# wearable-motion-capture/arm-pose-estimation

Measured on AMD Instinct MI355X. Metric: IMU windows/sec, higher is better.
Workload: dtype f32; 1 GPU; BASELINE configs[2]: watch_phone_pocket_lstm path, 1024 windows/GPU x 64 frames x 22 features (I=22,H=256,L=2,O=14), z-score+LSTM+head+denorm+FK, inputs resident in HBM; windows_per_gpu=1024, frames=64, features=22

## Files before the change

arm-pose-estimation_amd/csrc/lstm_cluster32.hip:

```cpp
#include <type_traits>

#include "ape_internal.h"
#include "async_look.h"
#include "../../include/ape_hip.h"

namespace {

typedef float f32x16 __attribute__((ext_vector_type(16)));
typedef unsigned u32x4 __attribute__((__vector_size__(4 * sizeof(unsigned))));
constexpr unsigned SPIN_LIMIT = 1u << 22;

#ifdef APE_CLUSTER_STAMPS
#define C32_TL(i) do { if (p.dbg_wg != nullptr && tid == 0 && cluster == 0 && member == 0 && (i) < 200) p.dbg_wg[256 + (i)] = __builtin_readcyclecounter(); } while (0)
#else
#define C32_TL(i) do {} while (0)
#endif

__device__ __forceinline__ float sigm(float v) { return __builtin_amdgcn_rcpf(1.0f + __builtin_amdgcn_exp2f(-1.4426950408889634f * v)); }
__device__ __forceinline__ float tanh_(float v) { return 2.0f * __builtin_amdgcn_rcpf(1.0f + __builtin_amdgcn_exp2f(-2.885390081777927f * v)) - 1.0f; }

template <bool AG>
__device__ __forceinline__ void mfma32(f32x16& acc, float w, float a) {
    if constexpr (AG) asm volatile("v_mfma_f32_32x32x2_f32 %0, %1, %2, %0" : "+v"(acc) : "a"(w), "v"(a));
    else asm volatile("v_mfma_f32_32x32x2_f32 %0, %1, %2, %0" : "+v"(acc) : "v"(w), "v"(a));
}
__device__ __forceinline__ void mfma_drain(f32x16& acc) { asm volatile("s_nop 15\n\ts_nop 7" : "+v"(acc)); }
template <bool AG>
__device__ __forceinline__ void mfma16(f32x16& acc, const u32x4& w, const u32x4& b) {
    if constexpr (AG) asm volatile("v_mfma_f32_32x32x16_f16 %0, %1, %2, %0" : "+v"(acc) : "a"(w), "v"(b));
    else asm volatile("v_mfma_f32_32x32x16_f16 %0, %1, %2, %0" : "+v"(acc) : "v"(w), "v"(b));
}

template <int NB, bool AG, int NW, typename Mid>
__device__ __forceinline__ void span32(f32x16& acc, const float* __restrict__ src, int stride, const float (&w)[NW], int w0, Mid&& mid) {
    f32x4 a0 = *reinterpret_cast<const f32x4*>(src);
    f32x4 a1 = (NB > 1) ? *reinterpret_cast<const f32x4*>(src + stride) : a0;
    f32x4 a2 = a1;
#pragma unroll
    for (int kb = 0; kb < NB; ++kb) {
        if (kb + 2 < NB) a2 = *reinterpret_cast<const f32x4*>(src + stride * (kb + 2));
#pragma unroll
        for (int j = 0; j < 4; ++j) mfma32<AG>(acc, w[w0 + 4 * kb + j], a0[j]);
        mid(kb);
        a0 = a1;
        a1 = a2;
    }
}

template <int NS, bool AG, int NG, typename Mid>
__device__ __forceinline__ void span16(f32x16& acc, const float* __restrict__ src, const u32x4 (&w)[NG], int g0, Mid&& mid) {
    constexpr int SL = 2 * 2 * 32 * 4;
    u32x4 h0 = *reinterpret_cast<const u32x4*>(src), l0 = *reinterpret_cast<const u32x4*>(src + 128);
    u32x4 h1 = (NS > 1) ? *reinterpret_cast<const u32x4*>(src + SL) : h0, l1 = (NS > 1) ? *reinterpret_cast<const u32x4*>(src + SL + 128) : l0;
    u32x4 h2 = h1, l2 = l1;
#pragma unroll
    for (int s = 0; s < NS; ++s) {
        if (s + 2 < NS) {
            h2 = *reinterpret_cast<const u32x4*>(src + SL * (s + 2));
            l2 = *reinterpret_cast<const u32x4*>(src + SL * (s + 2) + 128);
        }
        mfma16<AG>(acc, w[g0 + 2 * s], h0);
        mfma16<AG>(acc, w[g0 + 2 * s], l0);
        mid(2 * s);
        mfma16<AG>(acc, w[g0 + 2 * s + 1], h0);
        mid(2 * s + 1);
        h0 = h1; l0 = l1;
        h1 = h2; l1 = l2;
    }
}

template <bool HOT>
__device__ __forceinline__ void dma_1k(unsigned lds_addr, unsigned voff, u32x4 rsrc, unsigned soff, int piece_bytes) {
    if constexpr (HOT) {
        unsigned tmp;
        asm volatile("s_add_i32 m0, %1, %5\n\ts_add_i32 %0, %4, %5\n\tbuffer_load_dwordx4 %2, %3, %0 offen sc1 lds"
                     : "=&s"(tmp) : "s"(lds_addr), "v"(voff), "s"(rsrc), "s"(soff), "i"(piece_bytes) : "memory");
    } else {
        asm volatile("s_mov_b32 m0, %0\n\ts_nop 3\n\tbuffer_load_dwordx4 %1, %2, %3 offen sc1 lds"
                     :: "s"(lds_addr + (unsigned)piece_bytes), "v"(voff), "s"(rsrc), "s"(soff + (unsigned)piece_bytes) : "memory");
    }
}


#ifndef C32_QF
#define C32_QF 3
#endif
#ifndef C32_QPD
#define C32_QPD 0
#endif
#ifndef C32_XS
#define C32_XS 1
#endif
#ifndef C32_QFP
#define C32_QFP 12
#endif
#ifndef C32_QPX
#define C32_QPX 33
#endif
#ifndef C32_QJX
#define C32_QJX 54
#endif
#if defined(APE_C32_COUNTS) && defined(APE_C32_WAITS)
#error "APE_C32_COUNTS and APE_C32_WAITS write the same words of dbg_wg: one build, one of them"
#endif
template <int H, int L, int KX, bool ENDS, int BXU>
__global__ __launch_bounds__(256, 1) void ape_lstm_cluster32(const ClusterParams p) {
    constexpr int UPW = 8;
    constexpr int GH = H / (4 * UPW);
    constexpr int MR = 32;
    constexpr int SX = KX + 4;
    constexpr int BX = KX / 8, BH = H / 8;
    constexpr int NW0 = 4 * (BX + BH);
    constexpr int NW1 = 4 * (2 * BH);
    constexpr int NFL = 4 * GH;
    constexpr int HL = GH * 4 * MR * 8;
    constexpr int NDMA = HL * 4 / 1024 / 4;
    static_assert(H == 256 && L == 2 && KX == 32 && GH == 8 && NDMA == 8, "built for the 2 x 256 models");
    static_assert(BXU == BX || (BXU == BX - 1 && !ENDS), "the short-window instantiation keeps the four-block input span");

    const int tid = threadIdx.x;
    const int lane = tid & 63;
    const int wave = __builtin_amdgcn_readfirstlane(tid >> 6);
    const int n = lane & 31, hh = lane >> 5;
    const int T = p.T, I = p.I, O = p.O;
    const bool normalize = (p.flags & APE_FLAG_NORMALIZE_INPUT) != 0;
    const bool bcast_x = (p.flags & APE_FLAG_BROADCAST_X) != 0;

    extern __shared__ __attribute__((aligned(16))) float smem[];
    float* hb0 = smem;
    float* hb1 = hb0 + 2 * HL;
    float* xin = hb1 + HL;
    f32x4* bias_s = reinterpret_cast<f32x4*>(xin + 2 * MR * SX);
    f32x4* park_s = bias_s + 4 * L * 4 * 64;
    unsigned* look_s = reinterpret_cast<unsigned*>(park_s + 4 * 4 * 64);
    int* ctl = reinterpret_cast<int*>(look_s + 4 * 64);

    unsigned* const class_ticket = p.xcc_slots + 64;
    unsigned* const xcc_words = p.xcc_slots + 64 + 8 * 16;
    const int cls = blockIdx.x & 7;
    unsigned my_xcc;
    asm volatile("s_getreg_b32 %0, hwreg(HW_REG_XCC_ID)" : "=s"(my_xcc));
    my_xcc &= 0xFu;
    if (tid == 0) {
        ctl[0] = 0;
        ctl[1] = -1;
        if (__hip_atomic_load(p.status, __ATOMIC_RELAXED, __HIP_MEMORY_SCOPE_AGENT) == 0u) {
            const unsigned tk = __hip_atomic_fetch_add(class_ticket + cls * 16, 1u, __ATOMIC_RELAXED, __HIP_MEMORY_SCOPE_AGENT);
            if (tk < gridDim.x / 8) ctl[1] = (int)tk;
            else __hip_atomic_store(p.status, 2u, __ATOMIC_RELAXED, __HIP_MEMORY_SCOPE_AGENT);
        }
    }
    __syncthreads();
    if (ctl[1] < 0) return;
    const int ticket = __builtin_amdgcn_readfirstlane(ctl[1]);
    const int cluster = (ticket / GH) * 8 + cls, member = ticket % GH;
    const int row0 = cluster * MR;
    C32_TL(0);
    if (tid == 0)
        __hip_atomic_store(xcc_words + cluster * GH + member, 0x10u | my_xcc, __ATOMIC_RELAXED, __HIP_MEMORY_SCOPE_AGENT);

    constexpr int NE = (MR * KX) / 256;
    const int xk = tid % KX, xrow = tid / KX;
    const int rows_here = bcast_x ? MR : max(0, min(MR, p.B - row0));
    const unsigned long long x_addr = reinterpret_cast<unsigned long long>(p.x + (bcast_x ? (size_t)0 : (size_t)row0 * T * I));
    const unsigned x_lo = __builtin_amdgcn_readfirstlane((unsigned)x_addr), x_hi = __builtin_amdgcn_readfirstlane((unsigned)(x_addr >> 32));
    const int x_bytes = __builtin_amdgcn_readfirstlane((int)((size_t)(bcast_x ? 1 : rows_here) * T * I * sizeof(float)));
    const __amdgpu_buffer_rsrc_t x_rsrc = __builtin_amdgcn_make_buffer_rsrc(
        reinterpret_cast<float*>(((unsigned long long)x_hi << 32) | x_lo), 0, x_bytes, 0x00020000);
    const unsigned x_rowbytes = bcast_x ? 0u : (unsigned)(T * I * sizeof(float));
    const unsigned x_off0 = (xk < I) ? (unsigned)xrow * x_rowbytes + (unsigned)(xk * sizeof(float)) : 0x80000000u;
    const unsigned x_estride = (unsigned)(256 / KX) * x_rowbytes;
    float xr[NE];
    auto fetch_x = [&](int t) {
        const int slot = (t + p.x_ring >= T) ? t + p.x_ring - T : t + p.x_ring;
#pragma unroll
        for (int e = 0; e < NE; ++e) {
            const unsigned off = (xrow + e * (256 / KX) < rows_here) ? x_off0 + (unsigned)e * x_estride : 0x80000000u;
            xr[e] = __builtin_bit_cast(float, __builtin_amdgcn_raw_buffer_load_b32(x_rsrc, off, (unsigned)(slot * I * sizeof(float)), 0));
        }
    };
    double x_mean = (normalize && xk < I) ? p.xx_m[xk] : 0.0;
    double x_std = (normalize && xk < I) ? p.xx_s[xk] : 1.0;
    double x_rstd = (normalize && xk < I) ? p.xx_r[xk] : 1.0;
    asm volatile("" : "+v"(x_mean), "+v"(x_std), "+v"(x_rstd));
    auto stage_x = [&](int t) {
        float* const dst = xin + (ENDS ? 0 : (t & 1) * (MR * SX));
#pragma unroll
        for (int e = 0; e < NE; ++e) {
            const double d = (double)xr[e] - x_mean;
            const double q0 = d * x_rstd;
            const double rr = fma(-q0, x_std, d);
            const double q1 = fma(rr, x_rstd, q0);
            dst[(xrow + e * (256 / KX)) * SX + xk] = (float)((rr == rr) ? q1 : q0);
        }
    };
    constexpr int XA = ENDS ? 0 : 1;
    fetch_x(0);

    float w0[4 * BXU];
    u32x4 w0h[NW0 / 4 - BX];
    u32x4 w1[NW1 / 4];
    const f32x4* const s0 = reinterpret_cast<const f32x4*>(p.wcl[0]) + ((size_t)(member * 4 + wave) * (NW0 / 4)) * 64 + lane;
    const u32x4* const s1 = reinterpret_cast<const u32x4*>(p.wcl[1]) + ((size_t)(member * 4 + wave) * (NW1 / 4)) * 64 + lane;
#pragma unroll
    for (int i = 0; i < BXU; ++i) {
        const f32x4 v = s0[i * 64];
        w0[4 * i] = v[0]; w0[4 * i + 1] = v[1]; w0[4 * i + 2] = v[2]; w0[4 * i + 3] = v[3];
    }
    auto load_weights = [&]() {
#pragma unroll
        for (int i = BX; i < NW0 / 4; ++i) w0h[i - BX] = reinterpret_cast<const u32x4*>(s0)[i * 64];
#pragma unroll
        for (int i = 0; i < NW1 / 4; ++i) w1[i] = s1[i * 64];
    };
#pragma unroll
    for (int l = 0; l < L; ++l)
#pragma unroll
        for (int gate = 0; gate < 4; ++gate) {
            f32x4 bv;
#pragma unroll
            for (int j = 0; j < 4; ++j) bv[j] = p.bias[l][gate * H + member * 32 + wave * 8 + 4 * hh + j] * p.gate_scale[l];
            bias_s[((wave * L + l) * 4 + gate) * 64 + lane] = bv;
        }
    float cst[L][4];
#pragma unroll
    for (int l = 0; l < L; ++l)
#pragma unroll
        for (int j = 0; j < 4; ++j) cst[l][j] = 0.0f;

    const __amdgpu_buffer_rsrc_t hx_rsrc = __builtin_amdgcn_make_buffer_rsrc(p.hx, 0, (int)p.hx_bytes, 0x00020000);
    const unsigned long long hx_addr = reinterpret_cast<unsigned long long>(p.hx);
    u32x4 hx_desc;
    hx_desc[0] = __builtin_amdgcn_readfirstlane((unsigned)hx_addr);
    hx_desc[1] = __builtin_amdgcn_readfirstlane((unsigned)(hx_addr >> 32) & 0xFFFFu);
    hx_desc[2] = __builtin_amdgcn_readfirstlane((unsigned)p.hx_bytes);
    hx_desc[3] = 0x00020000u;
    unsigned* const flags_of = p.xflags + (size_t)cluster * L * NFL;
    const ape_desc_t fl_desc = ape_make_desc(p.xflags, (unsigned)((gridDim.x / GH) * L * NFL * sizeof(unsigned)));
    const unsigned fl_off = (unsigned)(cluster * L * NFL * sizeof(unsigned));
    const unsigned look_voff = (unsigned)((lane & (NFL - 1)) * sizeof(unsigned));
    const unsigned look_lds = (unsigned)reinterpret_cast<unsigned long long>(look_s) + (unsigned)(wave * 256);
    const unsigned* const look_mine = look_s + wave * 64 + lane;
    constexpr unsigned SET_BYTES = HL * sizeof(float);
    auto hx_base = [&](int l, int par) -> unsigned { return (unsigned)((((size_t)cluster * L + l) * 2 + par) * SET_BYTES); };
    const unsigned hb0_lds = (unsigned)reinterpret_cast<unsigned long long>(hb0);
    const unsigned hb1_lds = (unsigned)reinterpret_cast<unsigned long long>(hb1);

    stage_x(0);
    if (T > 1) fetch_x(1);

    if (wave == 0) {
        unsigned spins = 0, v = 0u;
        while (true) {
            v = 0x10u | my_xcc;
            if (lane < GH) v = __hip_atomic_load(xcc_words + cluster * GH + lane, __ATOMIC_RELAXED, __HIP_MEMORY_SCOPE_AGENT);
            if (__all((int)(v != 0u))) break;
            if (++spins > SPIN_LIMIT || __hip_atomic_load(p.status, __ATOMIC_RELAXED, __HIP_MEMORY_SCOPE_AGENT) != 0u) {
                if (lane == 0) {
                    ctl[0] = 1;
                    __hip_atomic_store(p.status, 1u, __ATOMIC_RELAXED, __HIP_MEMORY_SCOPE_AGENT);
                }
                break;
            }
            __builtin_amdgcn_s_sleep(2);
        }
        const int same = __all((int)((v & 0xFu) == my_xcc));
        if (lane == 0) ctl[3] = same;
    }
    __syncthreads();
    if (ctl[0] != 0) return;
    C32_TL(1);
    const bool in_l2 = APE_HANDOVER_IN_L2(p.flags, ctl[3] != 0);

    auto wait_flags = [&](int l, unsigned want) {
        unsigned spins = 0;
        while (true) {
            unsigned v = want;
            if (lane < NFL) v = __hip_atomic_load(flags_of + l * NFL + lane, __ATOMIC_RELAXED, __HIP_MEMORY_SCOPE_AGENT);
            if (__all((int)(v >= want))) return;
            if (++spins > SPIN_LIMIT || __hip_atomic_load(p.status, __ATOMIC_RELAXED, __HIP_MEMORY_SCOPE_AGENT) != 0u) {
                if (lane == 0) {
                    ctl[0] = 1;
                    __hip_atomic_store(p.status, 1u, __ATOMIC_RELAXED, __HIP_MEMORY_SCOPE_AGENT);
                }
                return;
            }
            __builtin_amdgcn_s_sleep(1);
        }
    };
    const unsigned dma_voff = (unsigned)(lane * 16);
    auto opaque = [](unsigned v) -> unsigned { asm volatile("" : "+s"(v)); return v; };
    const unsigned wave_kib = (unsigned)(wave * 1024);
    auto issue_piece = [&](auto hot_tag, int l, int step, int k) {
        constexpr bool HOT = decltype(hot_tag)::value;
        const unsigned wk = HOT ? wave_kib : opaque(wave_kib);
        const unsigned src = hx_base(l, step & 1) + wk;
        const unsigned dst = (l == 0 ? hb0_lds + (unsigned)((step & 1) * SET_BYTES) : hb1_lds) + wk;
        dma_1k<HOT>(dst, dma_voff, hx_desc, src, k * 4096);
    };
    constexpr std::true_type HOT{};
    constexpr std::false_type COLD{};
    int pend_idx = -1;
    unsigned pend_epoch = 0u;
    auto raise_pending = [&]() {
        if (pend_idx < 0) return;
        if (lane == 0) __hip_atomic_store(flags_of + pend_idx, pend_epoch, __ATOMIC_RELAXED, __HIP_MEMORY_SCOPE_AGENT);
        pend_idx = -1;
    };
    auto bar = [&]() { asm volatile("s_waitcnt lgkmcnt(0)\n\ts_barrier" ::: "memory"); };

    auto cell_update = [&](const f32x16& acc, int l, float (&c_)[4], float (&hn)[4]) {
        const float ks = -1.4426950408889634f * p.gate_descale[l], kt = -2.885390081777927f * p.gate_descale[l];
#pragma unroll
        for (int j = 0; j < 4; j += 2) {
            typedef float f32x2 __attribute__((ext_vector_type(2)));
            auto exp2_2 = [](f32x2 v) { return f32x2{__builtin_amdgcn_exp2f(v[0]), __builtin_amdgcn_exp2f(v[1])}; };
            auto rcp_2 = [](f32x2 v) { return f32x2{__builtin_amdgcn_rcpf(v[0]), __builtin_amdgcn_rcpf(v[1])}; };
            const f32x2 ai = {acc[j], acc[j + 1]}, af = {acc[4 + j], acc[5 + j]}, ag = {acc[8 + j], acc[9 + j]}, ao = {acc[12 + j], acc[13 + j]};
            const f32x2 iv = rcp_2(1.0f + exp2_2(ks * ai));
            const f32x2 fv = rcp_2(1.0f + exp2_2(ks * af));
            const f32x2 gv = 2.0f * rcp_2(1.0f + exp2_2(kt * ag)) - 1.0f;
            const f32x2 ov = rcp_2(1.0f + exp2_2(ks * ao));
            const f32x2 c = fv * f32x2{c_[j], c_[j + 1]} + iv * gv;
            c_[j] = c[0]; c_[j + 1] = c[1];
            const f32x2 h = ov * (2.0f * rcp_2(1.0f + exp2_2(-2.885390081777927f * c)) - 1.0f);
            hn[j] = h[0]; hn[j + 1] = h[1];
        }
    };
    const unsigned pub_off = (unsigned)((((member * 4 + wave) * MR + n) * 8 + 4 * hh) * sizeof(float));
    const unsigned pub_off_split = (unsigned)(((member * 4 + wave) * 2 * MR + hh * MR + n) * 16);
    auto split_h = [&](const float (&h)[4]) -> u32x4 {
        unsigned hw[2], lw[2];
#pragma unroll
        for (int d = 0; d < 2; ++d) {
            const float a = h[2 * d] * (float)(1 << APE_C32_HSHIFT), b = h[2 * d + 1] * (float)(1 << APE_C32_HSHIFT);
            const _Float16 ah = (_Float16)a, bh = (_Float16)b;
            const _Float16 al = (_Float16)(a - (float)ah), bl = (_Float16)(b - (float)bh);
            hw[d] = (unsigned)__builtin_bit_cast(unsigned short, ah) | ((unsigned)__builtin_bit_cast(unsigned short, bh) << 16);
            lw[d] = (unsigned)__builtin_bit_cast(unsigned short, al) | ((unsigned)__builtin_bit_cast(unsigned short, bl) << 16);
        }
        u32x4 r;
#pragma unroll
        for (int d = 0; d < 2; ++d) {
            const auto sw = __builtin_amdgcn_permlane32_swap(hw[d], lw[d], false, false);
            r[d] = sw[0];
            r[2 + d] = sw[1];
        }
        return r;
    };

    if constexpr (!ENDS) {
        if (1 < T) {
            stage_x(1);
            if (2 < T) fetch_x(2);
        }
        load_weights();
    } else {
        f32x16 acc;
#pragma unroll
        for (int gate = 0; gate < 4; ++gate) {
            const f32x4 bv = bias_s[((wave * L + 0) * 4 + gate) * 64 + lane];
            acc[4 * gate] = bv[0]; acc[4 * gate + 1] = bv[1]; acc[4 * gate + 2] = bv[2]; acc[4 * gate + 3] = bv[3];
        }
        span32<BXU, false, 4 * BXU>(acc, xin + n * SX + hh * 4, 8, w0, 0, [&](int) {});
        mfma_drain(acc);
        float h0[4];
        cell_update(acc, 0, cst[0], h0);
        const u32x4 hv = split_h(h0);
        if (in_l2) __builtin_amdgcn_raw_buffer_store_b128(hv, hx_rsrc, hx_base(0, 0) + pub_off_split, 0, 0);
        else __builtin_amdgcn_raw_buffer_store_b128(hv, hx_rsrc, hx_base(0, 0) + pub_off_split, 0, 16 );
        asm volatile("s_waitcnt vmcnt(0)" ::: "memory");
        if (lane == 0) __hip_atomic_store(flags_of + member * 4 + wave, 1u, __ATOMIC_RELAXED, __HIP_MEMORY_SCOPE_AGENT);
        asm volatile("" ::: "memory");
        load_weights();
        bar();
        if (1 < T) {
            stage_x(1);
            if (2 < T) fetch_x(2);
        }
    }
    C32_TL(2);

    const int P = T + L - 1;
    bool prefetched = false;
    bool parked = false;
#ifdef APE_C32_COUNTS
    unsigned lc_block[2] = {0u, 0u}, lc_go[2] = {0u, 0u}, lc_n[2] = {0u, 0u};
    unsigned long long lc_top[2] = {0ull, 0ull}, lc_t0 = 0ull;
    const unsigned long long lc_start = __builtin_amdgcn_s_memtime();
#endif
#ifdef APE_C32_WAITS
    unsigned long long lw[4] = {0ull, 0ull, 0ull, 0ull}, lw_t0 = 0ull;
    unsigned lw_n[3] = {0u, 0u, 0u};
    const unsigned long long lw_start = __builtin_amdgcn_s_memtime();
#define C32_WAIT_T0() do { if (ST) lw_t0 = __builtin_amdgcn_s_memtime(); } while (0)
#define C32_WAIT_T1(k) do { if (ST) lw[k] += __builtin_amdgcn_s_memtime() - lw_t0; } while (0)
#else
#define C32_WAIT_T0() do {} while (0)
#define C32_WAIT_T1(k) do {} while (0)
#endif
#ifdef APE_CLUSTER_STAMPS
    unsigned long long dg_block[2] = {0, 0}, dg_go[2] = {0, 0};
    unsigned long long dgh[2][6] = {};
    unsigned long long dgc[2][5] = {};
    auto now = [&]() -> unsigned long long {
        const unsigned long long c = __builtin_readcyclecounter();
        asm volatile("s_waitcnt lgkmcnt(0)" ::: "memory");
        return c;
    };
#endif
    auto section = [&](auto steady_tag, auto layer_tag, auto mode_tag, const int ph) -> bool {
        constexpr bool ST = decltype(steady_tag)::value;
        constexpr int l = decltype(layer_tag)::value;
        constexpr int MODE = decltype(mode_tag)::value;
        static_assert(MODE == 0 || (l == L - 1 && (MODE == 3 || !ST)), "the special forms are layer 1's");
        const int t = ph - l;
        const bool active = ST || (t >= 0 && t < T);
        const bool need = ST || (t >= 1 && t <= T);
#ifdef APE_CLUSTER_STAMPS
        const unsigned long long c0 = ST ? now() : 0ull;
#endif
#ifdef APE_C32_COUNTS
        lc_t0 = __builtin_amdgcn_s_memtime();
#endif
        if constexpr (MODE != 3) C32_WAIT_T0();
        if (MODE == 3) {
        } else if (need) {
            if (!prefetched) {
#ifdef APE_CLUSTER_STAMPS
                dg_block[l] += 1;
#endif
#ifdef APE_C32_COUNTS
                lc_block[l] += 1u;
#endif
                asm volatile("s_waitcnt vmcnt(0)" ::: "memory");
                raise_pending();
                wait_flags(l, (unsigned)t);
#pragma unroll
                for (int k = 0; k < NDMA; ++k) issue_piece(COLD, l, t - 1, k);
                asm volatile("s_waitcnt vmcnt(0)" ::: "memory");
            } else {
                asm volatile("s_waitcnt vmcnt(1)" ::: "memory");
            }
        }
        prefetched = false;
#ifdef APE_CLUSTER_STAMPS
        const unsigned long long c1 = ST ? now() : 0ull;
#endif
        if constexpr (MODE != 3) bar();
#ifdef APE_CLUSTER_STAMPS
        const unsigned long long c2 = ST ? now() : 0ull;
#endif
#ifdef APE_C32_COUNTS
        if (ST && MODE != 3) { lc_top[l] += __builtin_amdgcn_s_memtime() - lc_t0; lc_n[l] += 1u; }
#endif
#ifdef APE_C32_WAITS
        if constexpr (MODE != 3) { C32_WAIT_T1(3); if (ST) lw_n[1] += 1u; }
#endif
        const int abort_word = (MODE == 3) ? 0 : ctl[0];
        C32_TL(8 + 2 * (2 * ph + l));
        constexpr int ln = (l + 1 < L) ? l + 1 : 0;
        const int tn = (l + 1 < L) ? t - 1 : t + L;
        const bool pre = (l == L - 1) && (ST || (tn >= 1 && tn <= T));
        unsigned peek = (unsigned)tn;
        bool go = false;
        constexpr int NBL = (l == 0) ? BXU + BH : 2 * BH;
        constexpr bool LW = ST && !ENDS && MODE == 3;
        constexpr bool XS = LW && C32_XS != 0;
        constexpr int QF = (!ENDS && l == 0 && C32_XS != 0) ? (ST ? BXU + C32_QFP : (C32_QF > BXU ? C32_QF : BXU)) : C32_QF;
        constexpr int QP = (MODE == 1) ? 16 : LW ? C32_QPX : NBL / 2 - 2 + C32_QPD, QJ = (MODE == 1) ? 20 : LW ? C32_QJX : NBL / 2 + 2 + C32_QPD;
        static_assert(!LW || (QP >= 0 && QP < QJ - 1 && QJ + NDMA <= 2 * BH), "the look, its judge and the eight pieces fit the section");
        bool staged = false;
#ifdef APE_CLUSTER_STAMPS
        unsigned long long hk0 = 0, hk_free = 0;
#define HK_BEGIN() do { if (ST) hk0 = now(); } while (0)
#define HK_END(k) do { if (ST) dgh[l][k] += now() - hk0; } while (0)
#else
#define HK_BEGIN() do {} while (0)
#define HK_END(k) do {} while (0)
#endif
        auto mid = [&](int q) {
#ifdef APE_CLUSTER_STAMPS
            if (ST && q == QF + 2) hk_free = now();
            if (ST && q == QF + 10) dgh[l][5] += now() - hk_free;
#endif
            if (!XS && q == QF) {
                HK_BEGIN();
                asm volatile("s_waitcnt vmcnt(0)" ::: "memory");
                raise_pending();
                HK_END(0);
            }
            if (l == L - 1 && q == ((MODE == 3) ? BH + 1 : QF + 1) && (ST || ph + 1 + XA < T)) {
                HK_BEGIN();
                stage_x(ph + 1 + XA);
                if (ST || ph + 2 + XA < T) fetch_x(ph + 2 + XA);
                staged = true;
                HK_END(1);
            }
            if constexpr (l == L - 1) {
                if (q == QP) look_issue(look_lds, look_voff, fl_desc, fl_off + (unsigned)(ln * NFL * sizeof(unsigned)));
                if (q == QJ - 1) {
                    C32_WAIT_T0();
                    look_landed();
                    C32_WAIT_T1(1);
                    peek = *look_mine;
                }
                if (q == QJ) {
                    HK_BEGIN();
                    go = pre && __all((int)(peek >= (unsigned)tn)) != 0;
                    HK_END(2);
                }
                if (q >= QJ && q < QJ + NDMA && go) {
                    HK_BEGIN();
                    issue_piece(HOT, ln, tn - 1, q - QJ);
                    HK_END(3);
                }
            }
        };
        float hnew[4] = {0.0f, 0.0f, 0.0f, 0.0f};
        if (active) {
            if constexpr (XS) {
                look_issue(look_lds, look_voff, fl_desc, fl_off + (unsigned)(l * NFL * sizeof(unsigned)));
                f32x16 ax;
#pragma unroll
                for (int gate = 0; gate < 4; ++gate) {
                    const f32x4 bv = bias_s[((wave * L + 0) * 4 + gate) * 64 + lane];
                    ax[4 * gate] = bv[0]; ax[4 * gate + 1] = bv[1]; ax[4 * gate + 2] = bv[2]; ax[4 * gate + 3] = bv[3];
                }
                span32<BXU, false, 4 * BXU>(ax, xin + ((ph + 1) & 1) * (MR * SX) + n * SX + hh * 4, 8, w0, 0, [&](int) {});
                mfma_drain(ax);
#pragma unroll
                for (int gate = 0; gate < 4; ++gate)
                    park_s[(wave * 4 + gate) * 64 + lane] = f32x4{ax[4 * gate], ax[4 * gate + 1], ax[4 * gate + 2], ax[4 * gate + 3]};
                parked = true;
            }
            bool from_park = false;
            if constexpr (l == 0 && !ENDS) {
                from_park = parked;
                parked = false;
            }
            const f32x4* const start_s = from_park ? park_s + wave * 4 * 64 + lane : bias_s + (wave * L + l) * 4 * 64 + lane;
            f32x16 acc;
#pragma unroll
            for (int gate = 0; gate < 4; ++gate) {
                const f32x4 bv = start_s[gate * 64];
                acc[4 * gate] = bv[0]; acc[4 * gate + 1] = bv[1]; acc[4 * gate + 2] = bv[2]; acc[4 * gate + 3] = bv[3];
            }
            const int frag = hh * 2 * MR * 4 + n * 4;
            if constexpr (l == 0) {
                if (!from_park) span32<BXU, false, 4 * BXU>(acc, xin + (ENDS ? 0 : (t & 1) * (MR * SX)) + n * SX + hh * 4, 8, w0, 0, [&](int q) { mid(q); });
                if (ST || t > 0) span16<BH / 2, false, NW0 / 4 - BX>(acc, hb0 + ((t - 1) & 1) * HL + frag, w0h, 0, [&](int q) { mid(BXU + q); });
            } else if constexpr (MODE == 3) {
                constexpr int QO = QF + 1, QO2 = QO + 12;
                static_assert(XS || (QO2 + 4 + NDMA <= QP && (LW || QP < BH)), "the own gather's hooks sit in front of the look for the next section");
                unsigned pk = (unsigned)t;
                bool got1 = false, got2 = false;
                if constexpr (XS) {
                    C32_WAIT_T0();
                    look_landed();
                    C32_WAIT_T1(0);
                    raise_pending();
                    pk = *look_mine;
                    got1 = __all((int)(pk >= (unsigned)t)) != 0;
                    span16<BH / 2, true, NW1 / 4>(acc, hb0 + (t & 1) * HL + frag, w1, 0, [&](int q) {
                        mid(q);
                        if (q < NDMA && got1) issue_piece(HOT, l, t - 1, q);
                    });
                } else
                span16<BH / 2, true, NW1 / 4>(acc, hb0 + (t & 1) * HL + frag, w1, 0, [&](int q) {
                    mid(q);
                    if (q == QO) look_issue(look_lds, look_voff, fl_desc, fl_off + (unsigned)(l * NFL * sizeof(unsigned)));
                    if (q == QO + 3) {
                        C32_WAIT_T0();
                        look_landed();
                        C32_WAIT_T1(0);
                        pk = *look_mine;
                    }
                    if (q == QO + 4) got1 = __all((int)(pk >= (unsigned)t)) != 0;
                    if (q >= QO + 4 && q < QO + 4 + NDMA && got1) issue_piece(HOT, l, t - 1, q - (QO + 4));
                    if constexpr (!ST) {
                        if (q == QO2 && !got1) look_issue(look_lds, look_voff, fl_desc, fl_off + (unsigned)(l * NFL * sizeof(unsigned)));
                        if (q == QO2 + 3 && !got1) {
                            look_landed();
                            pk = *look_mine;
                        }
                        if (q == QO2 + 4 && !got1) got2 = __all((int)(pk >= (unsigned)t)) != 0;
                        if (q >= QO2 + 4 && q < QO2 + 4 + NDMA && got2) issue_piece(HOT, l, t - 1, q - (QO2 + 4));
                    }
                });
#ifdef APE_C32_COUNTS
                lc_t0 = __builtin_amdgcn_s_memtime();
#endif
                C32_WAIT_T0();
                if (!got1 && !got2) {
#ifdef APE_C32_WAITS
                    if (ST) lw_n[2] += 1u;
#endif
#ifdef APE_CLUSTER_STAMPS
                    dg_block[l] += 1;
#endif
#ifdef APE_C32_COUNTS
                    lc_block[l] += 1u;
#endif
                    asm volatile("s_waitcnt vmcnt(0)" ::: "memory");
                    raise_pending();
                    wait_flags(l, (unsigned)t);
#pragma unroll
                    for (int k = 0; k < NDMA; ++k) issue_piece(COLD, l, t - 1, k);
                }
                asm volatile("s_waitcnt vmcnt(0)" ::: "memory");
                bar();
#ifdef APE_C32_COUNTS
                if (ST) { lc_top[l] += __builtin_amdgcn_s_memtime() - lc_t0; lc_n[l] += 1u; }
#endif
#ifdef APE_C32_WAITS
                C32_WAIT_T1(2);
                if (ST) lw_n[0] += 1u;
#endif
                if (ctl[0] != 0) return false;
                span16<BH / 2, true, NW1 / 4>(acc, hb1 + frag, w1, BH, [&](int q) { mid(BH + q); });
            } else {
                span16<BH / 2, true, NW1 / 4>(acc, hb0 + (t & 1) * HL + frag, w1, 0, [&](int q) { mid(q); });
                if (ST || t > 0) span16<BH / 2, true, NW1 / 4>(acc, hb1 + frag, w1, BH, [&](int q) { mid(BH + q); });
            }
#ifdef APE_CLUSTER_STAMPS
            const unsigned long long c3 = ST ? now() : 0ull;
            if (ST) { dgc[l][0] += c1 - c0; dgc[l][1] += c2 - c1; dgc[l][2] += c3 - c2; }
#endif
            mfma_drain(acc);
            cell_update(acc, l, cst[l], hnew);
        }
        if (abort_word != 0) return false;
        if (!ST && pend_idx >= 0) {
            asm volatile("s_waitcnt vmcnt(0)" ::: "memory");
            raise_pending();
        }
        if (go) prefetched = true;
#ifdef APE_CLUSTER_STAMPS
        if (go) dg_go[ln] += 1;
#endif
#ifdef APE_C32_COUNTS
        if (go) lc_go[ln] += 1u;
#endif
        if constexpr (l == L - 1) {
            if (!ST && !staged && ph + 1 + XA < T) {
                stage_x(ph + 1 + XA);
                if (ph + 2 + XA < T) fetch_x(ph + 2 + XA);
            }
        }
        {
            const bool head_only = (l == L - 1) && !ST && t == T - 1;
            const u32x4 hs = split_h(hnew);
            const u32x4 hv = head_only ? u32x4{__builtin_bit_cast(unsigned, hnew[0]), __builtin_bit_cast(unsigned, hnew[1]),
                                               __builtin_bit_cast(unsigned, hnew[2]), __builtin_bit_cast(unsigned, hnew[3])} : hs;
            const unsigned off = active ? hx_base(l, t & 1) + (head_only ? pub_off : pub_off_split) : 0x80000000u;
            if (in_l2) __builtin_amdgcn_raw_buffer_store_b128(hv, hx_rsrc, off, 0, 0);
            else __builtin_amdgcn_raw_buffer_store_b128(hv, hx_rsrc, off, 0, 16 );
            if (active) {
                pend_idx = l * NFL + member * 4 + wave;
                pend_epoch = (unsigned)(t + 1);
            }
        }
#ifdef APE_CLUSTER_STAMPS
        if (ST) { dgc[l][3] += now() - c2; dgc[l][4] += 1; }
#endif
        C32_TL(9 + 2 * (2 * ph + l));
        return true;
    };
    bool ok = true;
#pragma unroll 1
    for (int ph = ENDS ? 1 : 0; ph < P && ok; ++ph) {
        const bool st0 = ph >= 2 && ph <= T - 3, st1 = st0;
        using M0 = std::integral_constant<int, 0>;
        using L0 = std::integral_constant<int, 0>;
        using L1 = std::integral_constant<int, 1>;
        ok = st0 ? section(std::true_type{}, L0{}, M0{}, ph) : section(std::false_type{}, L0{}, M0{}, ph);
        if (!ok) break;
        const int t1 = ph - 1;
        bool done1 = false;
        if constexpr (ENDS) {
            if (!st1 && t1 == 0 && T > 1) {
                ok = section(std::false_type{}, L1{}, std::integral_constant<int, 1>{}, ph);
                done1 = true;
            }
        }
        using M3 = std::integral_constant<int, 3>;
        if (!done1 && t1 >= 1 && t1 < T) {
            ok = st1 ? section(std::true_type{}, L1{}, M3{}, ph) : section(std::false_type{}, L1{}, M3{}, ph);
            done1 = true;
        }
        if (!done1) ok = section(std::false_type{}, L1{}, M0{}, ph);
    }
    if (!ok) return;
    {
        asm volatile("s_waitcnt vmcnt(0)" ::: "memory");
        bar();
        if (pend_idx >= 0) {
            if (wave == 0 && lane < 4)
                __hip_atomic_store(flags_of + (pend_idx - wave) + lane, pend_epoch, __ATOMIC_RELAXED, __HIP_MEMORY_SCOPE_AGENT);
            pend_idx = -1;
        }
        if (!prefetched) {
            wait_flags(L - 1, (unsigned)T);
#pragma unroll
            for (int k = 0; k < NDMA; ++k) issue_piece(COLD, L - 1, T - 1, k);
        }
        asm volatile("s_waitcnt vmcnt(0)" ::: "memory");
        bar();
        if (ctl[0] != 0) return;
        C32_TL(4);
    }

#ifdef APE_CLUSTER_STAMPS
    if (p.dbg_wg != nullptr && tid == 0 && cluster == 0 && member == 0)
        for (int k = 0; k < 2; ++k) { p.dbg_wg[16 + k] = dg_block[k]; p.dbg_wg[18 + k] = dg_go[k]; }
    if (p.dbg_wg != nullptr && lane == 0 && cluster == 0 && member == 0)
        for (int l = 0; l < 2; ++l)
            for (int k = 0; k < 5; ++k) p.dbg_wg[32 + wave * 16 + l * 5 + k] = dgc[l][k];
    if (p.dbg_wg != nullptr && lane == 0 && cluster == 0 && member == 0)
        for (int l = 0; l < 2; ++l)
            for (int k = 0; k < 6; ++k) p.dbg_wg[128 + wave * 16 + l * 6 + k] = dgh[l][k];
#endif
#ifdef APE_C32_COUNTS
    if (p.dbg_wg != nullptr && tid == 0 && cluster < 24) {
        unsigned long long* o = p.dbg_wg + 512 + (cluster * GH + member) * 8;
        o[0] = lc_block[0]; o[1] = lc_block[1]; o[2] = lc_go[0]; o[3] = lc_go[1];
        o[4] = lc_top[0]; o[5] = lc_top[1]; o[6] = lc_n[0]; o[7] = __builtin_amdgcn_s_memtime() - lc_start;
    }
#endif
#ifdef APE_C32_WAITS
    if (p.dbg_wg != nullptr && tid == 0 && cluster < 24) {
        unsigned long long* o = p.dbg_wg + 512 + (cluster * GH + member) * 8;
        o[0] = lw[0]; o[1] = lw[1]; o[2] = lw[2]; o[3] = lw[3];
        o[4] = lw_n[0]; o[5] = lw_n[1]; o[6] = lw_n[2]; o[7] = __builtin_amdgcn_s_memtime() - lw_start;
    }
#endif
    {
        constexpr int RPM = MR / GH;
        const int part = tid & 3;
        for (int oi = tid >> 2; oi < ((RPM * O + 63) / 64) * 64; oi += 64) {
            const bool live = oi < RPM * O;
            const int rr = live ? oi / O : 0, o = live ? oi - rr * O : 0;
            const int row = member * RPM + rr, b = row0 + row;
            float s_acc = 0.0f;
            if (live) {
                const float* wv = p.w_out + (size_t)o * H;
                for (int kb = part; kb < H / 8; kb += 4) {
                    const f32x4 a0 = *reinterpret_cast<const f32x4*>(hb1 + kb * MR * 8 + row * 8);
                    const f32x4 a1 = *reinterpret_cast<const f32x4*>(hb1 + kb * MR * 8 + row * 8 + 4);
                    const f32x4 u0 = *reinterpret_cast<const f32x4*>(wv + kb * 8), u1 = *reinterpret_cast<const f32x4*>(wv + kb * 8 + 4);
#pragma unroll
                    for (int j = 0; j < 4; ++j) s_acc = fmaf(a0[j], u0[j], s_acc);
#pragma unroll
                    for (int j = 0; j < 4; ++j) s_acc = fmaf(a1[j], u1[j], s_acc);
                }
            }
            s_acc += __shfl_xor(s_acc, 1, 64);
            s_acc += __shfl_xor(s_acc, 2, 64);
            if (p.y != nullptr && live && part == 0 && b < p.B) p.y[(size_t)b * O + o] = s_acc + p.b_out[o];
        }
    }
    C32_TL(5);
    __syncthreads();
    if (tid == 0)
        ctl[2] = (__hip_atomic_fetch_add(p.done, 1u, __ATOMIC_RELAXED, __HIP_MEMORY_SCOPE_AGENT) == gridDim.x - 1) ? 1 : 0;
    __syncthreads();
    if (ctl[2] != 0) {
        const int n_flags = (int)(gridDim.x / GH) * L * NFL;
        for (int i = tid; i < n_flags; i += 256) __hip_atomic_store(p.xflags + i, 0u, __ATOMIC_RELAXED, __HIP_MEMORY_SCOPE_AGENT);
        for (int i = tid; i < (int)gridDim.x; i += 256) __hip_atomic_store(xcc_words + i, 0u, __ATOMIC_RELAXED, __HIP_MEMORY_SCOPE_AGENT);
        if (tid < 8) __hip_atomic_store(class_ticket + tid * 16, 0u, __ATOMIC_RELAXED, __HIP_MEMORY_SCOPE_AGENT);
        if (tid == 0) __hip_atomic_store(p.done, 0u, __ATOMIC_RELAXED, __HIP_MEMORY_SCOPE_AGENT);
    }
}

constexpr size_t smem_bytes32() {
    return ((size_t)3 * 8 * 4 * 32 * 8 + (size_t)2 * 32 * 36) * sizeof(float) + (size_t)4 * (2 + 1) * 4 * 64 * 16 + (size_t)4 * 64 * sizeof(unsigned) + 16;
}

}

bool ape_cluster32_supported(int H, int L, int KX) { return H == 256 && L == 2 && KX == 32; }

hipError_t ape_prepare_lstm_cluster32(int H, int L, int KX) {
    if (!ape_cluster32_supported(H, L, KX)) return hipSuccess;
    static_assert(smem_bytes32() <= APE_LDS_BYTES, "LDS layout exceeds a CU");
    hipError_t e = hipFuncSetAttribute(reinterpret_cast<const void*>(&ape_lstm_cluster32<256, 2, 32, false, 3>),
                                       hipFuncAttributeMaxDynamicSharedMemorySize, APE_LDS_BYTES);
    if (e != hipSuccess) return e;
    e = hipFuncSetAttribute(reinterpret_cast<const void*>(&ape_lstm_cluster32<256, 2, 32, false, 4>),
                            hipFuncAttributeMaxDynamicSharedMemorySize, APE_LDS_BYTES);
    if (e != hipSuccess) return e;
    return hipFuncSetAttribute(reinterpret_cast<const void*>(&ape_lstm_cluster32<256, 2, 32, true, 4>),
                               hipFuncAttributeMaxDynamicSharedMemorySize, APE_LDS_BYTES);
}

hipError_t ape_launch_lstm_cluster32(int H, int L, int KX, int clusters, const ClusterParams& p, hipStream_t stream) {
    if (!ape_cluster32_supported(H, L, KX)) return hipErrorInvalidValue;
    const int grid_clusters = (clusters + 7) / 8 * 8;
    constexpr size_t smem = smem_bytes32();
    if (p.T <= APE_C32_ENDS_MAX_T) hipLaunchKernelGGL((ape_lstm_cluster32<256, 2, 32, true, 4>), dim3(grid_clusters * 8), dim3(256), smem, stream, p);
    else if (p.I <= 24) hipLaunchKernelGGL((ape_lstm_cluster32<256, 2, 32, false, 3>), dim3(grid_clusters * 8), dim3(256), smem, stream, p);
    else hipLaunchKernelGGL((ape_lstm_cluster32<256, 2, 32, false, 4>), dim3(grid_clusters * 8), dim3(256), smem, stream, p);
    return hipGetLastError();
}
```

Baseline: 3.136 million windows/s.

## Issue hidden-state DMA pieces unconditionally and raise flags with raw buffer stores

In the steady-state LSTM sections, the hidden-state DMA pieces are now always issued, with source and destination computed at the judge point, instead of only when the peer flags show readiness. Flag raises become inline buffer_store_dword instructions from a vector register with a precomputed offset, replacing the lane-0 atomic store. The goal is to remove the branchy readiness check and the scalar-to-vector traffic from the inter-workgroup handoff on the recurrent critical path. The risk is loading stale data speculatively, which is only safe if later flag checks still gate its use. A debug 'late' knob and asm markers are also added.

```diff
diff --git a/arm-pose-estimation_amd/csrc/lstm_cluster32.hip b/arm-pose-estimation_amd/csrc/lstm_cluster32.hip
--- a/arm-pose-estimation_amd/csrc/lstm_cluster32.hip
+++ b/arm-pose-estimation_amd/csrc/lstm_cluster32.hip
@@ -74,7 +74,7 @@
     if constexpr (HOT) {
         unsigned tmp;
         asm volatile("s_add_i32 m0, %1, %5\n\ts_add_i32 %0, %4, %5\n\tbuffer_load_dwordx4 %2, %3, %0 offen sc1 lds"
-                     : "=&s"(tmp) : "s"(lds_addr), "v"(voff), "s"(rsrc), "s"(soff), "i"(piece_bytes) : "memory");
+                     : "=&s"(tmp) : "s"(lds_addr), "v"(voff), "s"(rsrc), "s"(soff), "i"(piece_bytes) : "memory", "scc");
     } else {
         asm volatile("s_mov_b32 m0, %0\n\ts_nop 3\n\tbuffer_load_dwordx4 %1, %2, %3 offen sc1 lds"
                      :: "s"(lds_addr + (unsigned)piece_bytes), "v"(voff), "s"(rsrc), "s"(soff + (unsigned)piece_bytes) : "memory");
@@ -99,6 +99,15 @@
 #endif
 #ifndef C32_QJX
 #define C32_QJX 54
+#endif
+#ifndef C32_UG
+#define C32_UG 1
+#endif
+#ifndef C32_RS
+#define C32_RS 1
+#endif
+#ifndef APE_C32_LATE_EVERY
+#define APE_C32_LATE_EVERY 0
 #endif
 #if defined(APE_C32_COUNTS) && defined(APE_C32_WAITS)
 #error "APE_C32_COUNTS and APE_C32_WAITS write the same words of dbg_wg: one build, one of them"
@@ -294,17 +303,25 @@
     auto issue_piece = [&](auto hot_tag, int l, int step, int k) {
         constexpr bool HOT = decltype(hot_tag)::value;
         const unsigned wk = HOT ? wave_kib : opaque(wave_kib);
-        const unsigned src = hx_base(l, step & 1) + wk;
+        const unsigned src = ((HOT || ENDS) ? hx_base(l, step & 1) : opaque(hx_base(l, step & 1))) + wk;
         const unsigned dst = (l == 0 ? hb0_lds + (unsigned)((step & 1) * SET_BYTES) : hb1_lds) + wk;
         dma_1k<HOT>(dst, dma_voff, hx_desc, src, k * 4096);
     };
     constexpr std::true_type HOT{};
     constexpr std::false_type COLD{};
+    constexpr bool EV = !ENDS && C32_XS != 0 && C32_RS != 0;
     int pend_idx = -1;
-    unsigned pend_epoch = 0u;
+    unsigned pend_epoch = 0u, pend_epoch_v = 0u;
     auto raise_pending = [&]() {
         if (pend_idx < 0) return;
-        if (lane == 0) __hip_atomic_store(flags_of + pend_idx, pend_epoch, __ATOMIC_RELAXED, __HIP_MEMORY_SCOPE_AGENT);
+        if (lane == 0) __hip_atomic_store(flags_of + pend_idx, EV ? pend_epoch_v : pend_epoch, __ATOMIC_RELAXED, __HIP_MEMORY_SCOPE_AGENT);
+        pend_idx = -1;
+    };
+    const unsigned raise_voff = (lane == 0) ? (unsigned)((member * 4 + wave) * sizeof(unsigned)) : 0x80000000u;
+    auto raise_hot = [&](auto lo_tag) {
+        constexpr int lo = decltype(lo_tag)::value;
+        asm volatile("buffer_store_dword %0, %1, %2, %3 offen offset:%4 sc1"
+                     :: "v"(pend_epoch_v), "v"(raise_voff), "s"(fl_desc), "s"(fl_off), "i"(lo * NFL * (int)sizeof(unsigned)) : "memory");
         pend_idx = -1;
     };
     auto bar = [&]() { asm volatile("s_waitcnt lgkmcnt(0)\n\ts_barrier" ::: "memory"); };
@@ -415,6 +432,7 @@
         constexpr int MODE = decltype(mode_tag)::value;
         static_assert(MODE == 0 || (l == L - 1 && (MODE == 3 || !ST)), "the special forms are layer 1's");
         const int t = ph - l;
+        if constexpr (ST && !ENDS) asm volatile("; c32 steady section, layer %0: begin" :: "i"(l));
         const bool active = ST || (t >= 0 && t < T);
         const bool need = ST || (t >= 1 && t <= T);
 #ifdef APE_CLUSTER_STAMPS
@@ -470,6 +488,11 @@
         constexpr int QF = (!ENDS && l == 0 && C32_XS != 0) ? (ST ? BXU + C32_QFP : (C32_QF > BXU ? C32_QF : BXU)) : C32_QF;
         constexpr int QP = (MODE == 1) ? 16 : LW ? C32_QPX : NBL / 2 - 2 + C32_QPD, QJ = (MODE == 1) ? 20 : LW ? C32_QJX : NBL / 2 + 2 + C32_QPD;
         static_assert(!LW || (QP >= 0 && QP < QJ - 1 && QJ + NDMA <= 2 * BH), "the look, its judge and the eight pieces fit the section");
+        constexpr bool UG = LW && C32_UG != 0;
+        constexpr bool RS = ST && !ENDS && C32_XS != 0 && C32_RS != 0 && (l == 0 || XS);
+        constexpr int LATE = APE_C32_LATE_EVERY;
+        const bool late = LATE > 0 && ST && (ph % (LATE > 0 ? LATE : 1)) == 0;
+        unsigned ug_src = 0u, ug_dst = 0u;
         bool staged = false;
 #ifdef APE_CLUSTER_STAMPS
         unsigned long long hk0 = 0, hk_free = 0;
@@ -487,7 +510,8 @@
             if (!XS && q == QF) {
                 HK_BEGIN();
                 asm volatile("s_waitcnt vmcnt(0)" ::: "memory");
-                raise_pending();
+                if constexpr (RS) raise_hot(std::integral_constant<int, 1 - l>{});
+                else raise_pending();
                 HK_END(0);
             }
             if (l == L - 1 && q == ((MODE == 3) ? BH + 1 : QF + 1) && (ST || ph + 1 + XA < T)) {
@@ -507,10 +531,21 @@
                 }
                 if (q == QJ) {
                     HK_BEGIN();
-                    go = pre && __all((int)(peek >= (unsigned)tn)) != 0;
+                    go = pre && !late && __all((int)(peek >= (unsigned)tn)) != 0;
+                    if constexpr (UG) {
+                        ug_src = hx_base(ln, (tn - 1) & 1) + wave_kib;
+                        ug_dst = (hb1_lds + wave_kib) - (unsigned)((2 - ((tn - 1) & 1)) * SET_BYTES);
+                        asm volatile("" : "+s"(ug_src));
+                    }
                     HK_END(2);
                 }
-                if (q >= QJ && q < QJ + NDMA && go) {
+                if constexpr (UG) {
+                    if (q >= QJ && q < QJ + NDMA) {
+                        HK_BEGIN();
+                        dma_1k<true>(ug_dst, dma_voff, hx_desc, ug_src, (q - QJ) * 4096);
+                        HK_END(3);
+                    }
+                } else if (q >= QJ && q < QJ + NDMA && go) {
                     HK_BEGIN();
                     issue_piece(HOT, ln, tn - 1, q - QJ);
                     HK_END(3);
@@ -559,12 +594,17 @@
                     C32_WAIT_T0();
                     look_landed();
                     C32_WAIT_T1(0);
-                    raise_pending();
+                    if constexpr (RS) raise_hot(std::integral_constant<int, 1 - l>{});
+                    else raise_pending();
                     pk = *look_mine;
-                    got1 = __all((int)(pk >= (unsigned)t)) != 0;
+                    got1 = !late && __all((int)(pk >= (unsigned)t)) != 0;
+                    unsigned own_src = hx_base(l, (t - 1) & 1) + wave_kib;
+                    if constexpr (UG) asm volatile("" : "+s"(own_src));
                     span16<BH / 2, true, NW1 / 4>(acc, hb0 + (t & 1) * HL + frag, w1, 0, [&](int q) {
                         mid(q);
-                        if (q < NDMA && got1) issue_piece(HOT, l, t - 1, q);
+                        if constexpr (UG) {
+                            if (q < NDMA) dma_1k<true>(hb1_lds + wave_kib, dma_voff, hx_desc, own_src, q * 4096);
+                        } else if (q < NDMA && got1) issue_piece(HOT, l, t - 1, q);
                     });
                 } else
                 span16<BH / 2, true, NW1 / 4>(acc, hb0 + (t & 1) * HL + frag, w1, 0, [&](int q) {
@@ -576,7 +616,7 @@
                         C32_WAIT_T1(0);
                         pk = *look_mine;
                     }
-                    if (q == QO + 4) got1 = __all((int)(pk >= (unsigned)t)) != 0;
+                    if (q == QO + 4) got1 = !late && __all((int)(pk >= (unsigned)t)) != 0;
                     if (q >= QO + 4 && q < QO + 4 + NDMA && got1) issue_piece(HOT, l, t - 1, q - (QO + 4));
                     if constexpr (!ST) {
                         if (q == QO2 && !got1) look_issue(look_lds, look_voff, fl_desc, fl_off + (unsigned)(l * NFL * sizeof(unsigned)));
@@ -627,6 +667,7 @@
             const unsigned long long c3 = ST ? now() : 0ull;
             if (ST) { dgc[l][0] += c1 - c0; dgc[l][1] += c2 - c1; dgc[l][2] += c3 - c2; }
 #endif
+            if constexpr (ST && !ENDS) asm volatile("; c32 steady section, layer %0: end" :: "i"(l));
             mfma_drain(acc);
             cell_update(acc, l, cst[l], hnew);
         }
@@ -658,7 +699,10 @@
             else __builtin_amdgcn_raw_buffer_store_b128(hv, hx_rsrc, off, 0, 16 );
             if (active) {
                 pend_idx = l * NFL + member * 4 + wave;
-                pend_epoch = (unsigned)(t + 1);
+                if constexpr (EV) {
+                    pend_epoch_v = (unsigned)(t + 1);
+                    asm volatile("" : "+v"(pend_epoch_v));
+                } else pend_epoch = (unsigned)(t + 1);
             }
         }
 #ifdef APE_CLUSTER_STAMPS
@@ -697,7 +741,7 @@
         bar();
         if (pend_idx >= 0) {
             if (wave == 0 && lane < 4)
-                __hip_atomic_store(flags_of + (pend_idx - wave) + lane, pend_epoch, __ATOMIC_RELAXED, __HIP_MEMORY_SCOPE_AGENT);
+                __hip_atomic_store(flags_of + (pend_idx - wave) + lane, EV ? pend_epoch_v : pend_epoch, __ATOMIC_RELAXED, __HIP_MEMORY_SCOPE_AGENT);
             pend_idx = -1;
         }
         if (!prefetched) {
```

Measured after the change: 3.209 million windows/s (median of 6 runs). 1.02x the previous value.
